# SvenGronauer/phoenix-drone-simulation

Measured on AMD Instinct MI355X. Metric: env-steps/sec, higher is better.
Workload: dtype f32; 1 GPU; DroneHoverSimpleEnv-v0, 1048576 envs per GPU lockstep, fp32, observation noise off, thrust noise 0, domain randomisation -1, auto-reset on, action ring [64,N,4] = hover+0.0 + 0.1*N(0,1); envs_per_gpu=1048576, obs_dim=42, bytes_per_env_step=346, parallelism=env-shard x1, no data-path collective

## Files before the change

### include/pds.h

```cpp
#ifndef PDS_H
#define PDS_H

#include <stdint.h>

#ifdef __cplusplus
extern "C" {
#endif

#define PDS_VERSION 2

#define PDS_TASK_HOVER 0
#define PDS_TASK_CIRCLE 1
#define PDS_TASK_TAKEOFF 2

#define PDS_CTRL_PWM 0
#define PDS_CTRL_ATTITUDE_RATE 1
#define PDS_CTRL_ATTITUDE 2

#define PDS_MAX_LATENCY_STEPS 8
#define PDS_MAX_REF_POINTS 300

#define PDS_OK 0
#define PDS_EINVAL -1
#define PDS_ENODEVICE -2
#define PDS_EHIP -3
#define PDS_ENOMEM -4
#define PDS_EUNSUPPORTED -5

typedef struct pds_config {
  int32_t struct_size;
  int32_t task;
  int64_t num_envs;
  int64_t env_id_base;
  uint64_t seed;
  int32_t device;
  int32_t use_motor_dynamics;
  int32_t use_ground_effect;
  int32_t observation_noise;
  int32_t aggregate_phy_steps;
  int32_t enable_reset_distribution;
  int32_t max_episode_steps;
  int32_t auto_reset;
// ... 107 lines not shown
int pds_latency_steps(const pds_handle *h);

int pds_field_width(int field);
int pds_get_state(pds_handle *h, int field, void *d_out, void *stream);
int pds_set_state(pds_handle *h, int field, const void *d_in, void *stream);

int pds_count_nonfinite(pds_handle *h, int64_t *count, void *stream);

uint64_t pds_tick(const pds_handle *h);
uint64_t pds_sync_tick(pds_handle *h, void *stream);
int pds_set_tick(pds_handle *h, uint64_t tick);

int pds_bytes_per_env_step(const pds_handle *h);
int pds_bytes_per_env_step_k(const pds_handle *h, int k_steps);

const char *pds_last_error(const pds_handle *h);

int pds_philox4x32(const uint32_t *d_ctr, const uint32_t *d_key, int rounds, int64_t n, uint32_t *d_out, void *stream);

int pds_noise_normals(uint64_t seed, uint64_t tick, uint32_t block, uint64_t env_id_base, int64_t n, float *d_out, void *stream);

int pds_history_advance(int64_t n, int half, int history, const float *d_obs2, const uint8_t *d_terminated,
                        const uint8_t *d_truncated, const float *d_final_obs2, int auto_reset, const float *d_hist_in,
                        float *d_hist_out, float *d_final_hist, void *stream);

int pds_gae(const float *d_rew, const float *d_val, const uint8_t *d_terminated, const uint8_t *d_truncated,
            const float *d_final_val, const float *d_last_val, float gamma, float lam, float rew_scale,
            float rew_clip, int64_t T, int64_t N, float *d_adv, float *d_target_v, float *d_disc_ret,
            void *stream);

// ... 75 lines not shown
```

### phoenix-drone-simulation_amd/csrc/pds_api.hip

```cpp
#include <hip/hip_runtime.h>

#include <cmath>
#include <cstdarg>
#include <cstdio>
#include <cstdlib>
#include <cstring>
#include <new>
#include <utility>
#include <vector>

#include "pds_reset.h"

namespace pds {

struct FieldArgs {
  DevState st;
  Consts k;
  void *user;
  long long n;
  int field;
  int task;
  int set;
  int has_motor, has_dr, has_tn, has_on, ctrl;
  int regen_obs;
// ... 202 lines not shown
  DevState st;
  Consts k;
  LaunchFlags flags;
  int force_tile;
  float2 *d_circle_ref;
  void *slab;
  float4 *lat_buf;
  unsigned long long *d_count;
  unsigned long long *d_stamps;
  int obs_dim;
  int num_cus;
  uint64_t tick;
  bool was_reset;
  int stored_from_agg;
  bool split_reset;
  bool stored_ready;
  char err[512];
};

struct DeviceGuard {
  int prev = -1;
  bool switched = false;
  hipError_t err = hipSuccess;
  explicit DeviceGuard(int dev) {
    err = hipGetDevice(&prev);
    if (err == hipSuccess && prev != dev) {
      err = hipSetDevice(dev);
      switched = err == hipSuccess;
    }
  }
// ... 225 lines not shown
  h->cfg = *cfg;
  fill_consts(*cfg, h->k);
  h->obs_dim = obs_dim_of(*cfg);
  h->flags.motor = cfg->use_motor_dynamics != 0;
  h->flags.dr = cfg->domain_randomization > 0;
  h->flags.ge = cfg->use_ground_effect != 0;
  h->flags.tn = cfg->motor_thrust_noise > 0;
  h->flags.on = cfg->observation_noise > 0;
  h->flags.ctrl = cfg->control_mode;
  h->flags.lat = lat_steps > 0;
  h->flags.hold = h->k.obs_rate != 1;
  h->flags.half_tile = false;
  if (const char *ft = getenv("PDS_FORCE_TILE")) h->force_tile = (ft[0] == 'h') ? 1 : ((ft[0] == 'f') ? 2 : 0);
  h->split_reset = false;
  if (const char *sr = getenv("PDS_SPLIT_RESET")) h->split_reset = sr[0] == '1';
  h->stored_from_agg = PDS_STORED_OH_FROM_AGG;
  if (PDS_STORED_OH_FROM_AGG > 0)
    if (const char *sa = getenv("PDS_STORED_OH_FROM_AGG")) h->stored_from_agg = atoi(sa);
  const size_t n = (size_t)cfg->num_envs;
  const size_t ntiles = (n + kWave - 1) / kWave;
  const LaunchFlags &f = h->flags;
  DeviceGuard guard(cfg->device);
  hipError_t e = guard.err;
  if (e == hipSuccess) {
    hipDeviceProp_t prop;
    e = hipGetDeviceProperties(&prop, cfg->device);
    h->num_cus = (e == hipSuccess && prop.multiProcessorCount > 0) ? prop.multiProcessorCount : 256;
  }
  std::vector<std::pair<void **, size_t>> req;
  auto alloc = [&](void **p, size_t bytes) { req.emplace_back(p, bytes); };
// ... 1 lines not shown
  alloc((void **)&h->st.hist[0], n * 16); alloc((void **)&h->st.hist[1], n * 16);
  alloc((void **)&h->st.ctr, n * 4);
  alloc((void **)&h->st.clk, ntiles * sizeof(WaveClock));
  alloc((void **)&h->d_count, 256);
  if (f.motor) alloc((void **)&h->st.mx, n * 16);
  if (f.dr) { alloc((void **)&h->st.par0, n * 16); alloc((void **)&h->st.par1, n * 8); }
  if (f.dr && f.motor) { alloc((void **)&h->st.mA, n * 16); alloc((void **)&h->st.mK, n * 16); }
  if (f.tn) alloc((void **)&h->st.ou, n * 16);
  if (f.on) {
    alloc((void **)&h->st.nz0, n * 16); alloc((void **)&h->st.nz1, n * 8);
    alloc((void **)&h->st.oh0, n * 16); alloc((void **)&h->st.oh1, n * 16); alloc((void **)&h->st.oh2, n * 8);
  }
  if (f.ctrl >= 1) { alloc((void **)&h->st.pid0, n * 16); alloc((void **)&h->st.pid1, n * 8); }
  if (f.ctrl == 2) { alloc((void **)&h->st.pid2, n * 16); alloc((void **)&h->st.pid3, n * 8); }
  alloc((void **)&h->d_circle_ref, kRefPoints * sizeof(float2));
  {
    const size_t stagger = (size_t)kStaggerBytes;
    size_t total = 0;
    std::vector<size_t> off;
    for (size_t j = 0; j < req.size(); ++j) {
      total = (total + 255) / 256 * 256 + stagger;
      off.push_back(total);
      total += req[j].second;
    }
    if (e == hipSuccess) e = hipMalloc(&h->slab, total + 256);
    if (e == hipSuccess) e = hipMemset(h->slab, 0, total + 256);
    if (e == hipSuccess)
      for (size_t j = 0; j < req.size(); ++j) *req[j].first = (char *)h->slab + off[j];
  }
  if (e == hipSuccess) {
    float2 ref[kRefPoints];
    const int np = h->k.ref_points;
    for (int t = 0; t < kRefPoints; ++t) {
      const double ts = 2 * M_PI * (double)(t % np) / np;
      ref[t].x = (float)(0.25 * (1 - cos(ts)));
      ref[t].y = (float)(0.25 * sin(ts));
    }
    e = hipMemcpy(h->d_circle_ref, ref, sizeof(ref), hipMemcpyHostToDevice);
  }
  h->st.circle_ref = h->d_circle_ref;
  if (e == hipSuccess && h->flags.on) {
    hipLaunchKernelGGL(ctor_noise_kernel, dim3((unsigned)((n + 255) / 256)), dim3(256), 0, 0, h->st, (long long)n,
                       (unsigned long long)cfg->env_id_base, h->k.gyro_sb, (uint32_t)cfg->seed, (uint32_t)(cfg->seed >> 32));
    e = hipGetLastError();
  }
  if (e == hipSuccess) e = hipDeviceSynchronize();
  if (e != hipSuccess) {
    snprintf(g_create_err, sizeof(g_create_err), "allocation of %zu envs failed: %s", n, hipGetErrorString(e));
    pds_destroy(h);
    return e == hipErrorOutOfMemory ? PDS_ENOMEM : PDS_EHIP;
  }
  if (h->flags.lat) {
    const int rc = ensure_latency_buffer(h);
    if (rc != PDS_OK) {
      snprintf(g_create_err, sizeof(g_create_err), "%s", h->err);
      pds_destroy(h);
      return rc;
    }
  }
  *out = h;
  return PDS_OK;
}

extern "C" int pds_destroy(pds_handle *h) {
  if (!h) return PDS_OK;
  DeviceGuard guard(h->cfg.device);
  if (h->slab) (void)hipFree(h->slab);
  if (h->lat_buf) (void)hipFree(h->lat_buf);
  if (h->d_stamps) (void)hipFree(h->d_stamps);
  delete h;
  return PDS_OK;
}

extern "C" int pds_obs_dim(const pds_handle *h) { return h ? h->obs_dim : PDS_EINVAL; }
extern "C" int64_t pds_num_envs(const pds_handle *h) { return h ? h->cfg.num_envs : PDS_EINVAL; }
extern "C" uint64_t pds_tick(const pds_handle *h) { return h ? h->tick : 0; }
extern "C" int pds_latency_steps(const pds_handle *h) { return h ? h->k.lat_steps : PDS_EINVAL; }
extern "C" const char *pds_last_error(const pds_handle *h) { return h ? h->err : g_create_err; }

extern "C" uint64_t pds_sync_tick(pds_handle *h, void *stream) {
  if (!h) return 0;
  DeviceGuard guard(h->cfg.device);
  WaveClock c;
  if (hipStreamSynchronize((hipStream_t)stream) == hipSuccess &&
      hipMemcpy(&c, h->st.clk, sizeof(c), hipMemcpyDeviceToHost) == hipSuccess)
    h->tick = ((uint64_t)c.y << 32) | c.x;
// ... 161 lines not shown
  const unsigned cus = (unsigned)h->num_cus;
  lf.half_tile = grid.x > (unsigned)kFullTileBlocksPerCU * cus * (256 / kBlock) && grid.x <= (merged ? 5u : 8u) * cus * (256 / kBlock);
  if (h->force_tile) lf.half_tile = h->force_tile == 1;
  if (lf.on || lf.lat) lf.half_tile = false;
  int kind = kLaunchStep;
  if (PDS_REGEN_OBS && h->stored_from_agg > 0 && lf.on && !lf.hold && h->cfg.aggregate_phy_steps >= h->stored_from_agg &&
      d_variates == nullptr) {
    kind = kLaunchStepStored;
    if (!h->stored_ready) {
      if (const int rc = materialize_kept_obs(h, (hipStream_t)stream)) return rc;
      h->stored_ready = true;
    }
  }
  const bool split = h->split_reset && h->cfg.auto_reset && d_variates == nullptr && kind == kLaunchStep &&
                     split_reset_supported(h->cfg.task, lf);
  launch_family(h, split ? kLaunchStepSplit : kind, lf, grid, (hipStream_t)stream, a);
  if (split) {
    a.k_steps = lf.hold ? 2 : ((PDS_REGEN_OBS && lf.on) ? 0 : 1);
    const dim3 pgrid((unsigned)((a.n + kPostResetEnvsPerBlock - 1) / kPostResetEnvsPerBlock));
    launch_family(h, kLaunchPostReset, lf, pgrid, (hipStream_t)stream, a);
  }
  PDS_HIP(h, hipGetLastError());
  h->tick += 1;
  return PDS_OK;
}

extern "C" int pds_step(pds_handle *h, const float *d_actions, float *d_obs, float *d_reward,
                        uint8_t *d_terminated, uint8_t *d_truncated, float *d_cost, float *d_final_obs,
                        void *stream) {
  return pds_step_with_variates(h, d_actions, nullptr, d_obs, d_reward, d_terminated, d_truncated, d_cost,
                                d_final_obs, stream);
// ... 178 lines not shown
  DeviceGuard guard(h->cfg.device);
  PDS_HIP(h, guard.err);
  FieldArgs a;
  memset(&a, 0, sizeof(a));
  a.st = h->st; a.k = h->k; a.user = d_ptr; a.n = h->cfg.num_envs; a.field = field; a.task = h->cfg.task; a.set = set;
  a.has_motor = h->flags.motor; a.has_dr = h->flags.dr; a.has_tn = h->flags.tn; a.has_on = h->flags.on; a.ctrl = h->flags.ctrl;
  a.regen_obs = PDS_REGEN_OBS && h->flags.on && !h->flags.hold;
  if (set && field != PDS_F_NOISY_OBS)
    if (const int rc = materialize_kept_obs(h, (hipStream_t)stream)) return rc;
  a.env_id_base = (unsigned long long)h->cfg.env_id_base;
  a.seed_lo = (uint32_t)h->cfg.seed; a.seed_hi = (uint32_t)(h->cfg.seed >> 32);
  const dim3 grid((unsigned)((a.n + kBlock - 1) / kBlock));
  hipLaunchKernelGGL(field_kernel, grid, dim3(kBlock), 0, (hipStream_t)stream, a);
  PDS_HIP(h, hipGetLastError());
  if (set) h->was_reset = true;
  return PDS_OK;
}

extern "C" int pds_count_nonfinite(pds_handle *h, int64_t *count, void *stream) {
  if (!h || !count) return PDS_EINVAL;
  DeviceGuard guard(h->cfg.device);
  PDS_HIP(h, guard.err);
  hipStream_t s = (hipStream_t)stream;
  PDS_HIP(h, hipMemsetAsync(h->d_count, 0, sizeof(*h->d_count), s));
  const long long n = h->cfg.num_envs;
  hipLaunchKernelGGL(nonfinite_kernel, dim3((unsigned)((n + 255) / 256)), dim3(256), 0, s, h->st, n, h->d_count);
  PDS_HIP(h, hipGetLastError());
  unsigned long long host = 0;
  PDS_HIP(h, hipMemcpyAsync(&host, h->d_count, sizeof(host), hipMemcpyDeviceToHost, s));
  PDS_HIP(h, hipStreamSynchronize(s));
  *count = (int64_t)host;
  return PDS_OK;
}

extern "C" int pds_get_state(pds_handle *h, int field, void *d_out, void *stream) { return do_field(h, field, d_out, 0, stream); }
extern "C" int pds_set_state(pds_handle *h, int field, const void *d_in, void *stream) { return do_field(h, field, const_cast<void *>(d_in), 1, stream); }

template <int ROUNDS>
__global__ __launch_bounds__(256) void philox_kernel(const uint32_t *ctr, const uint32_t *key, long long n, uint32_t *out) {
  const long long i = (long long)blockIdx.x * blockDim.x + threadIdx.x;
  if (i >= n) return;
  const U4 r = philox4x32<ROUNDS>(ctr[4 * i], ctr[4 * i + 1], ctr[4 * i + 2], ctr[4 * i + 3], key[2 * i], key[2 * i + 1]);
  out[4 * i] = r.x; out[4 * i + 1] = r.y; out[4 * i + 2] = r.z; out[4 * i + 3] = r.w;
}

__global__ __launch_bounds__(256) void noise_normals_kernel(uint32_t seed_lo, uint32_t seed_hi, uint32_t tick_lo, uint32_t tick_hi,
                                                            uint32_t block, unsigned long long id_base, long long n, float *out) {
// ... 53 lines not shown
```

### phoenix-drone-simulation_amd/csrc/pds_reset.h

```cpp
#pragma once
#include "pds_types.h"

namespace pds {

constexpr uint32_t kBlkReset = 0;
constexpr uint32_t kBlkLatRows = 9;
constexpr uint32_t kBlkResetNoise = 32;
constexpr uint32_t kBlkObsNoise = 64;
constexpr uint32_t kBlkSubNoise = 128;
constexpr uint32_t kBlkSubNoiseX = 256;

constexpr int kResetBlocks = 9;
constexpr int kObsCallBlocks = 3;
constexpr int kResetNoiseBlocks = 2 * kObsCallBlocks;
constexpr int kLatRowBlocks = kMaxLatSteps - 1;
constexpr int kScratchBlocks = kResetBlocks + kResetNoiseBlocks + kLatRowBlocks;

PDS_DEV void words_to_uniforms4(const U4 &w, float (&u)[4]) {
  u[0] = u01(w.x); u[1] = u01(w.y); u[2] = u01(w.z); u[3] = u01(w.w);
}
PDS_DEV void words_to_normals4(const U4 &w, float (&z)[4]) {
  box_muller(w.x, w.y, z[0], z[1]);
  box_muller(w.z, w.w, z[2], z[3]);
}
// ... 691 lines not shown
    float stale_w[3] = {0.f, 0.f, 0.f}, bias[3] = {0.f, 0.f, 0.f};
    if (V::ON) {
      const float4 q2 = a.st.s2[i];
      const float4 nz = a.st.nz0[i];
      stale_w[0] = q2.y; stale_w[1] = q2.z; stale_w[2] = q2.w;
      bias[0] = nz.x; bias[1] = nz.y; bias[2] = nz.z;
    }
    ResetOut r;
    const DirectWords dw((uint32_t)(a.env_id_base + (unsigned long long)i), rk);
    const uint32_t ctr_old = ctr_pack(0u, 0u, circle_ref_offset(a.st.ctr[i], a.k.ref_points));
    reset_compute<V>(a, ref_lds, dw, ctr_old, a.samples != nullptr ? a.samples + i * PDS_SAMPLE_FLOATS : nullptr,
                     stale_w, bias, r);
    reset_store<V>(a, ref_lds, i, r);
  }
  advance_clock(a.st.clk, tile, rk, parity, 1u, threadIdx.x & (kWave - 1));
}

template <class V>
__global__ __launch_bounds__(kWave) void post_reset_kernel(const StepArgs a) {
  constexpr int D = V::D;
  constexpr int kPer = kPostResetEnvsPerBlock / kWave;
  static_assert(kPer == 16 || kPer == 8 || kPer == 4, "one 16- / 8- / 4-byte load of each flag array per lane");
  __shared__ uint32_t queue[kPostResetEnvsPerBlock];
  __shared__ int qn;
  const float2 *ref_lds = nullptr;
  const int lane = threadIdx.x;
  const long long base = (long long)blockIdx.x * kPostResetEnvsPerBlock;
  if (lane == 0) qn = 0;
  __builtin_amdgcn_fence(__ATOMIC_RELEASE, "workgroup");
  __builtin_amdgcn_wave_barrier();
// ... 13 lines not shown
    } else {
      for (int j = 0; j < kPer; ++j)
        if (e0 + j < a.n && (a.term[e0 + j] | a.trunc[e0 + j])) fl[j >> 2] |= 1u << (8 * (j & 3));
    }
    if ((fl[0] | fl[1] | fl[2] | fl[3]) != 0u) {
      int cnt = 0;
      for (int j = 0; j < kPer; ++j) cnt += ((fl[j >> 2] >> (8 * (j & 3))) & 0xFFu) != 0u;
      int at_ = atomicAdd(&qn, cnt);
      for (int j = 0; j < kPer; ++j)
        if (((fl[j >> 2] >> (8 * (j & 3))) & 0xFFu) != 0u) queue[at_++] = (uint32_t)(kPer * lane + j);
    }
  }
  __builtin_amdgcn_fence(__ATOMIC_RELEASE, "workgroup");
  __builtin_amdgcn_wave_barrier();
  __builtin_amdgcn_fence(__ATOMIC_ACQUIRE, "workgroup");
  const int n_fin = __builtin_amdgcn_readfirstlane(qn);
  for (int idx = lane; idx < n_fin; idx += kWave) {
    const long long i = base + queue[idx];
    const WaveClock clk = a.st.clk[i / kWave];
    RngKey rk{a.seed_lo, a.seed_hi, 0u, 0u};
    {
      const unsigned long long t = (((unsigned long long)clk.y << 32) | clk.x) - 1ull;
      rk.tick_lo = (uint32_t)t; rk.tick_hi = (uint32_t)(t >> 32);
    }
    if (a.final_obs != nullptr) {
      const float2 *src = reinterpret_cast<const float2 *>(a.obs + i * D);
      float2 *dst = reinterpret_cast<float2 *>(a.final_obs + i * D);
#pragma unroll
      for (int j = 0; j < D / 2; ++j) dst[j] = src[j];
    }
    float stale_w[3] = {0.f, 0.f, 0.f}, bias[3] = {0.f, 0.f, 0.f};
    if (V::ON) {
      const float4 q2 = a.st.s2[i];
      const float4 nz = a.st.nz0[i];
      stale_w[0] = q2.y; stale_w[1] = q2.z; stale_w[2] = q2.w;
      bias[0] = nz.x; bias[1] = nz.y; bias[2] = nz.z;
    }
    uint32_t ref_offset = 0u;
    if (V::TASK == PDS_TASK_CIRCLE && !a.k.reset_dist) ref_offset = circle_ref_offset(a.st.ctr[i], a.k.ref_points);
    ResetOut r;
    const DirectWords dw((uint32_t)(a.env_id_base + (unsigned long long)i), rk);
    reset_compute<V>(a, ref_lds, dw, ctr_pack(0u, 0u, ref_offset), nullptr, stale_w, bias, r);
    reset_store<V>(a, ref_lds, i, r, a.k_steps);
  }
}

}
```

### phoenix-drone-simulation_amd/csrc/pds_step.h

```cpp
#pragma once
#include <type_traits>
#include "pds_reset.h"

namespace pds {

template <int D>
constexpr int tile_stride() {
  return (D % 8 == 0) ? D + 4 : D;
}

template <int HW>
constexpr int park_stride() {
  return (HW % 4 == 0) ? ((HW / 4) % 2 == 1 ? HW : HW + 4) : (HW % 2 == 1 ? HW : HW + 1);
}

template <int N>
PDS_DEV void lds_store_row(float *dst, const float *src) {
  static_assert(N % 4 == 0, "float4 rows");
#pragma unroll
  for (int j = 0; j < N / 4; ++j)
    reinterpret_cast<float4 *>(dst)[j] = make_float4(src[4 * j], src[4 * j + 1], src[4 * j + 2], src[4 * j + 3]);
}

template <class V>
// ... 594 lines not shown
      S.oh.qx = fresh ? S.oh.qx : held.qx; S.oh.qy = fresh ? S.oh.qy : held.qy; S.oh.qz = fresh ? S.oh.qz : held.qz;
      S.oh.qw = fresh ? S.oh.qw : held.qw;
      S.oh.vx = fresh ? S.oh.vx : held.vx; S.oh.vy = fresh ? S.oh.vy : held.vy; S.oh.vz = fresh ? S.oh.vz : held.vz;
    }
    put_noisy_half<TASK, O + 4, VEC>(row2, S.oh, ns.lpf, act, tx, ty, tz, pa2);
  } else {
    put_obs_half<TASK, O + 4, VEC>(row2, e, q, act, tx, ty, tz, pa2);
  }

  S.ctr = ctr_pack((uint32_t)(step + 1), 0u, (uint32_t)phase1, lat_idx);
  if (regen_obs_variant<V>() && a.noise != nullptr) S.ctr |= kCtrOhBit;
  S.h2 = h1;
  S.h1 = act;
  const bool need_reset = (V::SPLIT_RESET && STORE) ? false : (a.auto_reset && (done || trunc) && active);
  const unsigned long long reset_mask = __ballot(need_reset);
  const unsigned long long done_mask = (a.final_obs != nullptr || fin_lds != nullptr) ? reset_mask : 0ull;
  if (so != nullptr) { so->reward = reward; so->done = done; so->trunc = trunc; }
  bool was_reset = false;
  if (reset_mask != 0ull) {
    const int pos = __builtin_amdgcn_mbcnt_hi((uint32_t)(reset_mask >> 32), __builtin_amdgcn_mbcnt_lo((uint32_t)reset_mask, 0u));
    if constexpr (RM == RM_DEFERRED) {
      qcount = __popcll(reset_mask);
      if (need_reset) queue[pos] = (uint32_t)lane | ((uint32_t)ref_offset << 6);
    } else if constexpr (RM == RM_MERGED) {
      const StepArgs &a = reload_args<101, heavy_variant<V>()>(a_in, (int)o1);
      const int count = __popcll(reset_mask);
      if (need_reset) queue[pos] = (uint32_t)lane;
      __builtin_amdgcn_fence(__ATOMIC_RELEASE, "wavefront");
      __builtin_amdgcn_wave_barrier();
      __builtin_amdgcn_fence(__ATOMIC_ACQUIRE, "wavefront");
      float4 u0 = act, mxr = make_float4(xm[0], xm[1], xm[2], xm[3]);
// ... 189 lines not shown
  return was_reset;
}

#ifndef PDS_MIN_WAVES_LEAN
#define PDS_MIN_WAVES_LEAN 4
#endif
#ifndef PDS_MIN_WAVES
#define PDS_MIN_WAVES (V::ON ? (four_block_variant<V>() ? 4 : 3) : PDS_MIN_WAVES_LEAN)
#endif

template <class V, int TR>
constexpr bool inline_reset_single_step() {
  return TR == kWave && inline_single_step_rule(V::TASK, V::ON, V::LAT, V::CTRL);
}

#ifndef PDS_MERGED_HALF_PT1DR
#define PDS_MERGED_HALF_PT1DR 1
#endif
template <class V, int TR = kWave>
constexpr bool merged_reset_variant() {
  return PDS_MERGED_RESET && !V::ON && !V::LAT && V::TASK != PDS_TASK_TAKEOFF && (TR == kWave || !(V::MOTOR && V::DR) || (PDS_MERGED_HALF_PT1DR && V::CTRL == 0 && !V::TN));
}

#ifndef PDS_KERNARG_PREFETCH
#define PDS_KERNARG_PREFETCH 1
#endif
PDS_DEV void prefetch_kernargs() {
#if PDS_KERNARG_PREFETCH
  static_assert(sizeof(StepArgs) > 8 * 64 && sizeof(StepArgs) <= 9 * 64, "prefetch_kernargs touches lines 0..8: adjust");
  const auto p = __builtin_amdgcn_kernarg_segment_ptr();
// ... 47 lines not shown
#ifdef PDS_STAMPS
#define PDS_STAMP_ARG , stamp_
#define PDS_STAMP_DECL unsigned long long stamp_[kStampSlots] = {0, 0, 0, 0, 0, 0, 0, 0, 0, 0}; stamp_[0] = __builtin_amdgcn_s_memtime(); stamp_[8] = __builtin_amdgcn_s_memrealtime();
#define PDS_STAMP_FLUSH                                                                                \
  do {                                                                                                 \
    PDS_STAMP_WAIT(7);                                                                                 \
    stamp_[9] = __builtin_amdgcn_s_memrealtime();                                                      \
    if (a.stamps != nullptr && lane == 0)                                                              \
      for (int j_ = 0; j_ < kStampSlots; ++j_) a.stamps[t * kStampSlots + j_] = stamp_[j_];            \
  } while (0)
#else
#define PDS_STAMP_ARG
#define PDS_STAMP_DECL
#define PDS_STAMP_FLUSH do { } while (0)
#endif

template <class V, int TR>
__global__ __launch_bounds__(kBlock, (PDS_MIN_WAVES) * (256 / kBlock)) void step_kernel(const StepArgs a) {
  PDS_STAMP_DECL
  prefetch_kernargs();
  constexpr int RM = merged_reset_variant<V, TR>() ? RM_MERGED : (inline_reset_single_step<V, TR>() ? RM_INLINE : RM_DEFERRED);
  PDS_WAVE_SETUP(V, TR, RM, true)
  Loaded cur;
  load_env<V>(a, ix, t, cur);
  __builtin_amdgcn_sched_barrier(0);
  PDS_STAMP(1);
  PDS_STAMP_WAIT(2);
  RngKey rk{a.seed_lo, a.seed_hi, 0u, 0u};
  int parity;
  rk.tick_lo = (uint32_t)__builtin_amdgcn_readfirstlane((int)cur.clk.x);
  rk.tick_hi = (uint32_t)__builtin_amdgcn_readfirstlane((int)cur.clk.y);
  parity = __builtin_amdgcn_readfirstlane((int)cur.clk.z) & 1;
  EnvState S;
  unpack_state<V>(a.k, cur, parity, S);
  init_kept_obs<V>(a, rk, ix, S);
  int qcount = 0;
  step_once<V, TR, RM, true>(a, 0ll, rk, parity, ref_lds, tile, park, queue, scratch, lane, wave_base, ix, active, cur.act, S, qcount, nullptr, nullptr PDS_STAMP_ARG);
  if (RM == RM_DEFERRED && qcount > 0) {
    const float own_w[3] = {S.e.wx, S.e.wy, S.e.wz};
    drain_reset_queue<V>(reload_args<104, heavy_variant<V>()>(a), rk, ref_lds, queue, qcount, lane, wave_base, tile, own_w, S.ns.bias);
  }
  PDS_STAMP(6);
  advance_clock(reload_args<105, heavy_variant<V>()>(a).st.clk, t, rk, parity ^ 1, 1u, lane);
  PDS_STAMP_FLUSH;
}

#ifndef PDS_STEPK_OPAQUE_KEY
#define PDS_STEPK_OPAQUE_KEY 1
#endif
#ifndef PDS_STEPK_MIN_WAVES_OF
#define PDS_STEPK_MIN_WAVES_OF(V) 3
#endif
template <class V_>
__global__ __launch_bounds__(kBlock, (PDS_STEPK_MIN_WAVES_OF(V_)) * (256 / kBlock)) void step_k_kernel(const StepArgs a) {
  using W = std::conditional_t<regen_obs_variant<V_>(), StoredOh<V_>, V_>;
  constexpr int TR = kWave;
  constexpr int RM = merged_reset_variant<W>() ? RM_MERGED : RM_INLINE;
#ifdef PDS_STAMPS
// ... 47 lines not shown
  } else {
#if PDS_STORED_OH_FROM_AGG > 0
    if constexpr (regen_obs_variant<V>()) {
      if (kind == kLaunchStepStored) {
        hipLaunchKernelGGL((step_kernel<StoredOh<V>, kWave>), grid, dim3(kBlock), 0, s, a);
        return;
      }
    }
#endif
    if constexpr (!V::ON && !V::LAT) {
      if (half_tile) {
        hipLaunchKernelGGL((step_kernel<V, kHalfTileRows>), grid, dim3(kBlock), 0, s, a);
        return;
      }
    }
    if constexpr (inline_reset_single_step<V, kWave>()) {
      if (kind == kLaunchStepSplit) {
        hipLaunchKernelGGL((step_kernel<SplitReset<V>, kWave>), grid, dim3(kBlock), 0, s, a);
        return;
      }
    }
    hipLaunchKernelGGL((step_kernel<V, kWave>), grid, dim3(kBlock), 0, s, a);
  }
}

template <int TASK, int CTRL, bool LAT, bool HOLD, bool MOTOR, bool DR, bool GE, bool TN, bool ON>
struct MakeVariant {
  using type = Variant<TASK, MOTOR, DR, GE, TN, ON, CTRL, LAT, HOLD>;
};

// ... 80 lines not shown
```

### phoenix-drone-simulation_amd/csrc/pds_types.h

```cpp
#pragma once
#include <hip/hip_runtime.h>
#include <stddef.h>
#include <stdint.h>

#include "../../include/pds.h"
#include "pds_device.h"

namespace pds {

#ifndef PDS_BLOCK
#define PDS_BLOCK 256
#endif
constexpr int kBlock = PDS_BLOCK;
#ifndef PDS_MERGED_RESET
#define PDS_MERGED_RESET 1
#endif
constexpr int kWave = 64;
constexpr int kHalfTileRows = 32;
constexpr int kFullTileBlocksPerCU = 3;
constexpr int kQueueCap = 64;
constexpr int kRefPoints = 300;
constexpr int kStaggerBytes = 4352;

constexpr int kStampSlots = 10;
// ... 103 lines not shown
  int ref_points;
  float ref_dth_hi, ref_dth_lo;
  int obs_rate;
};

struct StepArgs {
  DevState st;
  Consts k;
  const float4 *actions;
  float *obs;
  float *reward;
  uint8_t *term;
  uint8_t *trunc;
  float *cost;
  float *final_obs;
  const uint8_t *mask;
  const float *samples;
  const float *noise;
  long long n;
  unsigned long long env_id_base;
  uint32_t seed_lo, seed_hi;
  int auto_reset;
  int k_steps;
  unsigned long long *stamps;
};

#ifndef PDS_RELOAD_ARGS
#define PDS_RELOAD_ARGS 1
#endif
template <int ID, bool ENABLE = true>
PDS_DEV const StepArgs &reload_args(const StepArgs &passed, int tag = 0) {
  if (!ENABLE || !PDS_RELOAD_ARGS) return passed;
// ... 10 lines not shown
struct Variant {
  static constexpr bool HOLD = HOLD_;
  static constexpr int CTRL = CTRL_;
  static constexpr bool LAT = LAT_;
  static constexpr int TASK = TASK_;
  static constexpr bool MOTOR = MOTOR_;
  static constexpr bool DR = DR_;
  static constexpr bool GE = GE_;
  static constexpr bool TN = TN_;
  static constexpr bool ON = ON_;
  static constexpr int O = ON_ ? (TASK_ == PDS_TASK_HOVER ? 13 : (TASK_ == PDS_TASK_CIRCLE ? 16 : 20))
                               : (TASK_ == PDS_TASK_HOVER ? 17 : (TASK_ == PDS_TASK_CIRCLE ? 16 : 20));
  static constexpr int D = 2 * (O + 4);
  static constexpr bool OH_STORED = false;
  static constexpr bool SPLIT_RESET = false;
};

template <class V>
struct StoredOh : V {
  static constexpr bool OH_STORED = true;
};

template <class V>
struct SplitReset : V {
  static constexpr bool SPLIT_RESET = true;
};

struct EnvRegs {
  float px, py, pz, vx, vy, vz, roll, pitch, yaw, wx, wy, wz;
};

struct Params {
  float dt, m, Jx, Jy, Jz, ftf1;
  float A[4], K[4];
};

struct ObsNoise {
  float pos_z[3], pos_u[3], vel_z[3], bias_z[3], rw_z[3], to_z[3], th_z[3], th_u[3];
};

// ... 53 lines not shown
  int ctrl;
  bool lat;
  bool hold;
  bool half_tile;
};
#ifndef PDS_STORED_OH_FROM_AGG
#define PDS_STORED_OH_FROM_AGG 0
#endif
#ifndef PDS_INLINE_SINGLE_STEP
#define PDS_INLINE_SINGLE_STEP 1
#endif
constexpr bool inline_single_step_rule(int task, bool on, bool lat, int ctrl) {
  return PDS_INLINE_SINGLE_STEP && (on || lat) && task != PDS_TASK_TAKEOFF && !(task == PDS_TASK_CIRCLE && (lat || ctrl != 0));
}
inline bool split_reset_supported(int task, const LaunchFlags &f) { return inline_single_step_rule(task, f.on, f.lat, f.ctrl); }
enum LaunchKind { kLaunchStep = 0, kLaunchStepK = 1, kLaunchReset = 2, kLaunchStepStored = 3, kLaunchStepSplit = 4, kLaunchPostReset = 5 };
#ifndef PDS_POST_RESET_ENVS
#define PDS_POST_RESET_ENVS 1024
#endif
constexpr int kPostResetEnvsPerBlock = PDS_POST_RESET_ENVS;
struct RolloutArgs {
  StepArgs s;
  pds_mlp pi, vf;
  const float *mean, *stdv;
  float eps;
  const float *log_std;
  unsigned long long seed;
  const unsigned long long *call_base;
  unsigned long long call_offset;
  int deterministic, T;
  const float *obs0;
  float *act_buf, *logp_buf, *val_buf, *fval_buf, *last_val;
  float *ep_ret, *ep_len, *stats;
};

// ... 62 lines not shown
```

### phoenix-drone-simulation_amd/envs.py

```python
import contextlib
import ctypes as C
import sys

import numpy as np
import torch

from . import native

_NULL_CTX = contextlib.nullcontext()

try:
    from gymnasium.spaces import Box as _GymBox
except Exception:
    _GymBox = None


_RAW_STREAM = getattr(torch._C, "_cuda_getCurrentRawStream", None)

class Box:

    def __init__(self, low, high, dtype=np.float32):
        self.low = np.asarray(low, dtype=dtype)
        self.high = np.asarray(high, dtype=dtype)
        self.shape = self.low.shape
# ... 369 lines not shown
    def set_state(self, name, value):
        fid = native.FIELDS[name]
        w = self.lib.pds_field_width(fid)
        dt = torch.int32 if name in native.INT_FIELDS else torch.float32
        v = torch.as_tensor(value).to(device=self.device, dtype=dt).reshape(self.num_envs, w).contiguous()
        rc = self.lib.pds_set_state(self._handle, fid, C.c_void_p(v.data_ptr()), self._stream())
        native.check(self._handle, rc, f"pds_set_state({name})")
        torch.cuda.current_stream(self.device).synchronize()

    def count_nonfinite(self):
        out = C.c_int64(0)
        rc = self.lib.pds_count_nonfinite(self._handle, C.byref(out), self._stream())
        native.check(self._handle, rc, "pds_count_nonfinite")
        return int(out.value)

    def state_dict(self):
        sd = {name: self.get_state(name) for name in native.FIELDS if name != "quat"}
        sd["tick"] = int(self.tick)
        if self._hist is not None:
            sd["observation_history"] = self._hist.clone()
        return sd

    def load_state_dict(self, sd):
        for name, v in sd.items():
            if name == "observation_history":
                self._hist = v.to(self.device).clone()
            elif name != "tick":
                self.set_state(name, v)
        rc = self.lib.pds_set_tick(self._handle, int(sd["tick"]))
        native.check(self._handle, rc, "pds_set_tick")
# ... 49 lines not shown
```

### phoenix-drone-simulation_amd/native.py

```python
import ctypes as C
import os

from .build import library_path

TASK_HOVER, TASK_CIRCLE, TASK_TAKEOFF = 0, 1, 2
OK, EINVAL, ENODEVICE, EHIP, ENOMEM, EUNSUPPORTED = 0, -1, -2, -3, -4, -5
SAMPLE_FLOATS = 112
MAX_LATENCY_STEPS = 8
NOISE_FLOATS = 52
FIELDS = dict(pos=0, rpy=1, vel=2, omega=3, quat=4, motor_x=5, last_action=6, prev_action=7,
              step_count=8, quat_sign=9, ref_offset=10, params=11, motor_A=12, motor_K=13, ou=14,
              gyro_bias=15, gyro_lpf=16, noisy_obs=17, pid=18, action_buffer=19, action_idx=20)
CONTROL_MODES = {'PWM': 0, 'AttitudeRate': 1, 'Attitude': 2}
INT_FIELDS = ("step_count", "quat_sign", "ref_offset", "action_idx")
SAMPLE_LAYOUT = dict(pos_offset=(0, 3), rpy=(3, 3), vel=(6, 3), omega=(9, 3), motor_x=(12, 4),
                     action=(16, 4), dr_dt=(20, 1), dr_m=(21, 1), dr_J=(22, 3), dr_ftf0=(25, 1),
                     dr_ftf1=(26, 1), dr_T=(27, 4), dr_t2w=(31, 4), ref_offset=(35, 1),
                     noise_call0=(36, 24), noise_call1=(60, 24), action_buf=(84, 28))
OBS_NOISE_LAYOUT = dict(pos_z=0, pos_u=3, vel_z=6, bias_z=9, rw_z=12, to_z=15, th_z=18, th_u=21)
STEP_NOISE_LAYOUT = dict(ou=0, a_bias=4, a_rw=7, a_to=10, obs=13, a_pos_z=37, a_pos_u=40, a_vel_z=43, a_th_z=46, a_th_u=49)

EXPORTS = ["pds_version", "pds_default_config", "pds_create", "pds_destroy", "pds_obs_dim",
           "pds_num_envs", "pds_reset", "pds_reset_from_samples", "pds_step", "pds_step_with_variates",
           "pds_field_width",
           "pds_get_state", "pds_set_state", "pds_tick", "pds_set_tick", "pds_sync_tick", "pds_count_nonfinite",
           "pds_bytes_per_env_step", "pds_bytes_per_env_step_k", "pds_last_error", "pds_step_k", "pds_set_latency",
           "pds_latency_steps", "pds_philox4x32", "pds_noise_normals", "pds_gae", "pds_history_advance",
           "pds_mlp_param_count", "pds_mlp_workspace_floats", "pds_mlp_forward", "pds_ppo_policy_grad",
           "pds_value_grad", "pds_ppo_policy_grad_step", "pds_value_grad_step", "pds_gaussian_sample", "pds_gaussian_sample_dev", "pds_counter_add", "pds_permutation", "pds_rollout_record",
           "pds_adam_step", "pds_rollout", "pds_rollout_history",
           "pds_npg_workspace_floats", "pds_npg_fisher_vector_product", "pds_npg_cg_step", "pds_npg_surrogate_kl"]


class Mlp(C.Structure):
    _fields_ = [("d_in", C.c_int32), ("h1", C.c_int32), ("h2", C.c_int32), ("d_out", C.c_int32),
                ("activation", C.c_int32),
                ("w1", C.c_void_p), ("b1", C.c_void_p), ("w2", C.c_void_p), ("b2", C.c_void_p),
                ("w3", C.c_void_p), ("b3", C.c_void_p)]


class Adam(C.Structure):
    _fields_ = [("d_exp_avg", C.c_void_p), ("d_exp_avg_sq", C.c_void_p), ("step", C.c_int64),
                ("lr", C.c_float), ("beta1", C.c_float), ("beta2", C.c_float), ("eps", C.c_float)]


class Config(C.Structure):
# ... 81 lines not shown

    later("pds_ppo_policy_grad_step", [mp, vp, vp, vp, vp, vp, i64, C.c_float, vp, vp, vp, ap, vp])
    later("pds_value_grad_step", [mp, vp, vp, vp, i64, vp, vp, vp, ap, vp])
    later("pds_gaussian_sample_dev", [vp, vp, i64, i32, u64, vp, u64, u64, i32, vp, vp, vp])
    later("pds_counter_add", [vp, u64, vp])
    later("pds_noise_normals", [u64, u64, C.c_uint32, u64, i64, vp, vp])
    later("pds_permutation", [vp, i64, u64, u64, vp])
    later("pds_rollout", [vp, i32, mp, mp, vp, vp, C.c_float, vp, u64, vp, u64, i32] + [vp] * 14)
    later("pds_rollout_history", [vp, i32, i32, mp, vp, vp, C.c_float, vp, u64, vp, u64, i32] + [vp] * 9 + [i32] + [vp] * 4)
    later("pds_npg_workspace_floats", [mp, i32])
    if hasattr(lib, "pds_npg_workspace_floats"):
        lib.pds_npg_workspace_floats.restype = i64
    later("pds_npg_fisher_vector_product", [mp, vp, vp, i64, vp, vp, C.c_float, vp, vp, vp])
    later("pds_npg_cg_step", [i64, vp, vp, vp, vp, vp, C.c_float, C.c_float, i32, vp])
    later("pds_npg_surrogate_kl", [mp, vp, vp, i32] + [vp] * 6 + [i64, vp, vp, vp, vp])
    _lib = lib
    return lib


def default_config(task):
    cfg = Config()
    rc = load().pds_default_config(int(task), C.byref(cfg))
    if rc != OK:
        raise ValueError(f"pds_default_config({task}) -> {rc}")
    return cfg


def check(handle, rc, what):
    if rc == OK:
        return
# ... 5 lines not shown
```

Before: 18.98 billion env-steps/s.

## Add group-wide deferred reset drained by last wave via cross-block counters

Adds a GroupReset step variant, on by default for hover tasks without latency or control. After stepping, each wave publishes its finished-env mask to global memory and bumps a per-group atomic counter, with dense waves resetting their own envs. One drainer wave per 1024-env group spins on the counter, collects the masks and resets all finished envs of the group. This moves the divergent reset work out of the hot step path and balances it across lanes, at the cost of inter-block polling, global atomics and a stall watchdog reported through pinned host memory.

```diff
diff --git a/include/pds.h b/include/pds.h
--- a/include/pds.h
+++ b/include/pds.h
@@ -26,6 +26,7 @@
 #define PDS_EHIP -3
 #define PDS_ENOMEM -4
 #define PDS_EUNSUPPORTED -5
+#define PDS_ESTALLED -6
 
 typedef struct pds_config {
   int32_t struct_size;
@@ -163,6 +164,8 @@
 int pds_bytes_per_env_step(const pds_handle *h);
 int pds_bytes_per_env_step_k(const pds_handle *h, int k_steps);
 
+uint32_t pds_device_status(const pds_handle *h);
+
 const char *pds_last_error(const pds_handle *h);
 
 int pds_philox4x32(const uint32_t *d_ctr, const uint32_t *d_key, int rounds, int64_t n, uint32_t *d_out, void *stream);
diff --git a/phoenix-drone-simulation_amd/csrc/pds_api.hip b/phoenix-drone-simulation_amd/csrc/pds_api.hip
--- a/phoenix-drone-simulation_amd/csrc/pds_api.hip
+++ b/phoenix-drone-simulation_amd/csrc/pds_api.hip
@@ -240,6 +240,9 @@
   bool was_reset;
   int stored_from_agg;
   bool split_reset;
+  bool group_reset;
+  uint32_t *group_sync;
+  volatile uint32_t *group_status;
   bool stored_ready;
   char err[512];
 };
@@ -495,6 +498,8 @@
   if (const char *ft = getenv("PDS_FORCE_TILE")) h->force_tile = (ft[0] == 'h') ? 1 : ((ft[0] == 'f') ? 2 : 0);
   h->split_reset = false;
   if (const char *sr = getenv("PDS_SPLIT_RESET")) h->split_reset = sr[0] == '1';
+  h->group_reset = PDS_GROUP_RESET_DEFAULT != 0;
+  if (const char *gr = getenv("PDS_GROUP_RESET")) h->group_reset = gr[0] == '1';
   h->stored_from_agg = PDS_STORED_OH_FROM_AGG;
   if (PDS_STORED_OH_FROM_AGG > 0)
     if (const char *sa = getenv("PDS_STORED_OH_FROM_AGG")) h->stored_from_agg = atoi(sa);
@@ -526,6 +531,7 @@
   if (f.ctrl >= 1) { alloc((void **)&h->st.pid0, n * 16); alloc((void **)&h->st.pid1, n * 8); }
   if (f.ctrl == 2) { alloc((void **)&h->st.pid2, n * 16); alloc((void **)&h->st.pid3, n * 8); }
   alloc((void **)&h->d_circle_ref, kRefPoints * sizeof(float2));
+  alloc((void **)&h->group_sync, group_sync_bytes((long long)n));
   {
     const size_t stagger = (size_t)kStaggerBytes;
     size_t total = 0;
@@ -551,6 +557,14 @@
     e = hipMemcpy(h->d_circle_ref, ref, sizeof(ref), hipMemcpyHostToDevice);
   }
   h->st.circle_ref = h->d_circle_ref;
+  if (e == hipSuccess) {
+    void *p = nullptr;
+    e = hipHostMalloc(&p, 64, hipHostMallocDefault);
+    if (e == hipSuccess) {
+      h->group_status = (volatile uint32_t *)p;
+      *h->group_status = 0u;
+    }
+  }
   if (e == hipSuccess && h->flags.on) {
     hipLaunchKernelGGL(ctor_noise_kernel, dim3((unsigned)((n + 255) / 256)), dim3(256), 0, 0, h->st, (long long)n,
                        (unsigned long long)cfg->env_id_base, h->k.gyro_sb, (uint32_t)cfg->seed, (uint32_t)(cfg->seed >> 32));
@@ -580,8 +594,20 @@
   if (h->slab) (void)hipFree(h->slab);
   if (h->lat_buf) (void)hipFree(h->lat_buf);
   if (h->d_stamps) (void)hipFree(h->d_stamps);
+  const bool stalled = h->group_status != nullptr && *h->group_status != 0u;
+  if (h->group_status) (void)hipHostFree((void *)h->group_status);
   delete h;
-  return PDS_OK;
+  return stalled ? PDS_ESTALLED : PDS_OK;
+}
+
+extern "C" uint32_t pds_device_status(const pds_handle *h) { return (h && h->group_status) ? *h->group_status : 0u; }
+
+static int group_status_check(pds_handle *h) {
+  const uint32_t w = pds_device_status(h);
+  if (w == 0u) return PDS_OK;
+  return fail(h, PDS_ESTALLED, "pds_step: the reset drainer of env group %u (envs %llu...) gave up waiting for the group's waves; "
+              "its finished envs were not reset (PDS_GROUP_RESET=0 selects the in-place reset)", w - 1u,
+              (unsigned long long)(w - 1u) * kPostResetEnvsPerBlock);
 }
 
 extern "C" int pds_obs_dim(const pds_handle *h) { return h ? h->obs_dim : PDS_EINVAL; }
@@ -773,7 +799,13 @@
   }
   const bool split = h->split_reset && h->cfg.auto_reset && d_variates == nullptr && kind == kLaunchStep &&
                      split_reset_supported(h->cfg.task, lf);
-  launch_family(h, split ? kLaunchStepSplit : kind, lf, grid, (hipStream_t)stream, a);
+  const bool group = !split && h->group_reset && h->cfg.auto_reset && d_variates == nullptr && kind == kLaunchStep &&
+                     group_reset_supported(h->cfg.task, lf);
+  if (group) {
+    a.group_sync = h->group_sync;
+    a.group_status = const_cast<uint32_t *>(h->group_status);
+  }
+  launch_family(h, split ? kLaunchStepSplit : (group ? kLaunchStepGroup : kind), lf, grid, (hipStream_t)stream, a);
   if (split) {
     a.k_steps = lf.hold ? 2 : ((PDS_REGEN_OBS && lf.on) ? 0 : 1);
     const dim3 pgrid((unsigned)((a.n + kPostResetEnvsPerBlock - 1) / kPostResetEnvsPerBlock));
@@ -982,7 +1014,7 @@
   hipLaunchKernelGGL(field_kernel, grid, dim3(kBlock), 0, (hipStream_t)stream, a);
   PDS_HIP(h, hipGetLastError());
   if (set) h->was_reset = true;
-  return PDS_OK;
+  return set ? PDS_OK : group_status_check(h);
 }
 
 extern "C" int pds_count_nonfinite(pds_handle *h, int64_t *count, void *stream) {
@@ -998,7 +1030,7 @@
   PDS_HIP(h, hipMemcpyAsync(&host, h->d_count, sizeof(host), hipMemcpyDeviceToHost, s));
   PDS_HIP(h, hipStreamSynchronize(s));
   *count = (int64_t)host;
-  return PDS_OK;
+  return group_status_check(h);
 }
 
 extern "C" int pds_get_state(pds_handle *h, int field, void *d_out, void *stream) { return do_field(h, field, d_out, 0, stream); }
diff --git a/phoenix-drone-simulation_amd/csrc/pds_reset.h b/phoenix-drone-simulation_amd/csrc/pds_reset.h
--- a/phoenix-drone-simulation_amd/csrc/pds_reset.h
+++ b/phoenix-drone-simulation_amd/csrc/pds_reset.h
@@ -729,6 +729,40 @@
     reset_store<V>(a, ref_lds, i, r);
   }
   advance_clock(a.st.clk, tile, rk, parity, 1u, threadIdx.x & (kWave - 1));
+}
+
+template <class V, bool COPY_FINAL>
+PDS_DEV void post_reset_serve(const StepArgs &a, const float2 *ref_lds, long long base, const uint32_t *queue, int n_fin, int lane,
+                              int oh_mode) {
+  constexpr int D = V::D;
+  for (int idx = lane; idx < n_fin; idx += kWave) {
+    const long long i = base + queue[idx];
+    const WaveClock clk = a.st.clk[i / kWave];
+    RngKey rk{a.seed_lo, a.seed_hi, 0u, 0u};
+    {
+      const unsigned long long t = (((unsigned long long)clk.y << 32) | clk.x) - 1ull;
+      rk.tick_lo = (uint32_t)t; rk.tick_hi = (uint32_t)(t >> 32);
+    }
+    if (COPY_FINAL && a.final_obs != nullptr) {
+      const float2 *src = reinterpret_cast<const float2 *>(a.obs + i * D);
+      float2 *dst = reinterpret_cast<float2 *>(a.final_obs + i * D);
+#pragma unroll
+      for (int j = 0; j < D / 2; ++j) dst[j] = src[j];
+    }
+    float stale_w[3] = {0.f, 0.f, 0.f}, bias[3] = {0.f, 0.f, 0.f};
+    if (V::ON) {
+      const float4 q2 = a.st.s2[i];
+      const float4 nz = a.st.nz0[i];
+      stale_w[0] = q2.y; stale_w[1] = q2.z; stale_w[2] = q2.w;
+      bias[0] = nz.x; bias[1] = nz.y; bias[2] = nz.z;
+    }
+    uint32_t ref_offset = 0u;
+    if (V::TASK == PDS_TASK_CIRCLE && !a.k.reset_dist) ref_offset = circle_ref_offset(a.st.ctr[i], a.k.ref_points);
+    ResetOut r;
+    const DirectWords dw((uint32_t)(a.env_id_base + (unsigned long long)i), rk);
+    reset_compute<V>(a, ref_lds, dw, ctr_pack(0u, 0u, ref_offset), nullptr, stale_w, bias, r);
+    reset_store<V>(a, ref_lds, i, r, oh_mode);
+  }
 }
 
 template <class V>
@@ -772,35 +806,7 @@
   __builtin_amdgcn_fence(__ATOMIC_RELEASE, "workgroup");
   __builtin_amdgcn_wave_barrier();
   __builtin_amdgcn_fence(__ATOMIC_ACQUIRE, "workgroup");
-  const int n_fin = __builtin_amdgcn_readfirstlane(qn);
-  for (int idx = lane; idx < n_fin; idx += kWave) {
-    const long long i = base + queue[idx];
-    const WaveClock clk = a.st.clk[i / kWave];
-    RngKey rk{a.seed_lo, a.seed_hi, 0u, 0u};
-    {
-      const unsigned long long t = (((unsigned long long)clk.y << 32) | clk.x) - 1ull;
-      rk.tick_lo = (uint32_t)t; rk.tick_hi = (uint32_t)(t >> 32);
-    }
-    if (a.final_obs != nullptr) {
-      const float2 *src = reinterpret_cast<const float2 *>(a.obs + i * D);
-      float2 *dst = reinterpret_cast<float2 *>(a.final_obs + i * D);
-#pragma unroll
-      for (int j = 0; j < D / 2; ++j) dst[j] = src[j];
-    }
-    float stale_w[3] = {0.f, 0.f, 0.f}, bias[3] = {0.f, 0.f, 0.f};
-    if (V::ON) {
-      const float4 q2 = a.st.s2[i];
-      const float4 nz = a.st.nz0[i];
-      stale_w[0] = q2.y; stale_w[1] = q2.z; stale_w[2] = q2.w;
-      bias[0] = nz.x; bias[1] = nz.y; bias[2] = nz.z;
-    }
-    uint32_t ref_offset = 0u;
-    if (V::TASK == PDS_TASK_CIRCLE && !a.k.reset_dist) ref_offset = circle_ref_offset(a.st.ctr[i], a.k.ref_points);
-    ResetOut r;
-    const DirectWords dw((uint32_t)(a.env_id_base + (unsigned long long)i), rk);
-    reset_compute<V>(a, ref_lds, dw, ctr_pack(0u, 0u, ref_offset), nullptr, stale_w, bias, r);
-    reset_store<V>(a, ref_lds, i, r, a.k_steps);
-  }
-}
-
-}
+  post_reset_serve<V, true>(a, ref_lds, base, queue, __builtin_amdgcn_readfirstlane(qn), lane, a.k_steps);
+}
+
+}
diff --git a/phoenix-drone-simulation_amd/csrc/pds_step.h b/phoenix-drone-simulation_amd/csrc/pds_step.h
--- a/phoenix-drone-simulation_amd/csrc/pds_step.h
+++ b/phoenix-drone-simulation_amd/csrc/pds_step.h
@@ -632,7 +632,9 @@
   S.h1 = act;
   const bool need_reset = (V::SPLIT_RESET && STORE) ? false : (a.auto_reset && (done || trunc) && active);
   const unsigned long long reset_mask = __ballot(need_reset);
-  const unsigned long long done_mask = (a.final_obs != nullptr || fin_lds != nullptr) ? reset_mask : 0ull;
+  constexpr bool kGroupForm = V::GROUP_RESET && STORE;
+  const unsigned long long fin_rows = kGroupForm ? __ballot(a.auto_reset && (done || trunc) && active) : reset_mask;
+  const unsigned long long done_mask = (a.final_obs != nullptr || fin_lds != nullptr) ? fin_rows : 0ull;
   if (so != nullptr) { so->reward = reward; so->done = done; so->trunc = trunc; }
   bool was_reset = false;
   if (reset_mask != 0ull) {
@@ -852,6 +854,11 @@
   return TR == kWave && inline_single_step_rule(V::TASK, V::ON, V::LAT, V::CTRL);
 }
 
+template <class V>
+constexpr bool group_reset_variant() {
+  return group_reset_rule(V::TASK, V::ON, V::LAT, V::CTRL, V::HOLD);
+}
+
 #ifndef PDS_MERGED_HALF_PT1DR
 #define PDS_MERGED_HALF_PT1DR 1
 #endif
@@ -929,6 +936,94 @@
 #define PDS_STAMP_DECL
 #define PDS_STAMP_FLUSH do { } while (0)
 #endif
+
+template <class V, int LDS_WORDS>
+PDS_DEV void group_reset_tail(const StepArgs &a, long long tile_index, long long ntiles, int lane, bool fin, uint32_t *lds) {
+  static_assert(LDS_WORDS > kPostResetEnvsPerBlock, "the queue of a group + its count live in the wave's observation tile");
+  constexpr int GT = kGroupTiles, WPB = kBlock / kWave, BPG = GT / WPB;
+  using RV = Variant<V::TASK, V::MOTOR, V::DR, false, false, V::ON, 0, V::LAT, false>;
+  const int oh_mode = V::HOLD ? 2 : ((PDS_REGEN_OBS && V::ON) ? 0 : 1);
+  const unsigned long long fin_mask = __ballot(fin);
+  const int n_own = __popcll(fin_mask);
+  const uint32_t t = (uint32_t)__builtin_amdgcn_readfirstlane((int)tile_index);
+  const uint32_t nt = (uint32_t)ntiles;
+  const uint32_t g = t / GT, blk = t / WPB, blk0 = g * BPG;
+  const uint32_t nb = gridDim.x, b = blockIdx.x;
+  const int nblk = (int)min((uint32_t)BPG, nb - blk0), j_own = (int)(blk - blk0);
+  bool last_block = j_own == nblk - 1;
+  if (PDS_XCD_REMAP && nb % 8u == 0u) {
+    const int per = (int)(nb / 8u);
+    last_block = true;
+    for (int j = 0; j < nblk; ++j) {
+      int y = (int)(b / 8u) + (j - j_own), x = (int)(b % 8u);
+      while (y >= per) { y -= per; ++x; }
+      while (y < 0) { y += per; --x; }
+      if ((uint32_t)(8 * y + x) > b) last_block = false;
+    }
+  }
+  const int tiles_here = (int)min((uint32_t)GT, nt - g * GT);
+  const bool drainer = last_block && (t % WPB) == min((uint32_t)(WPB - 1), nt - 1u - blk * WPB);
+  uint32_t *const counter = a.group_sync + (size_t)g * kGroupCounterStride;
+  unsigned long long *const masks =
+      reinterpret_cast<unsigned long long *>(a.group_sync + (size_t)((nt + GT - 1) / GT) * kGroupCounterStride) + (size_t)g * GT;
+  unsigned long long m = 0ull;
+  long long base;
+  if (!drainer) {
+    const bool dense = n_own >= kGroupDenseFrom;
+    if (n_own != 0 && !dense) {
+      if (lane == 0) masks[t % GT] = fin_mask;
+      asm volatile("s_waitcnt vmcnt(0)" ::: "memory");
+      __builtin_amdgcn_fence(__ATOMIC_RELEASE, "agent");
+      asm volatile("s_waitcnt vmcnt(0)" ::: "memory");
+    }
+    if (lane == 0) (void)__hip_atomic_fetch_add(counter, 1u, __ATOMIC_RELAXED, __HIP_MEMORY_SCOPE_AGENT);
+    if (!dense) return;
+    asm volatile("s_waitcnt vmcnt(0)" ::: "memory");
+    if (lane == 0) m = fin_mask;
+    base = (long long)t * kWave;
+  } else {
+    const uint32_t expected = (uint32_t)tiles_here - 1u;
+    uint32_t seen = 0u;
+    for (int it = 0; expected != 0u; ++it) {
+      seen = (uint32_t)__builtin_amdgcn_readfirstlane((int)__hip_atomic_load(counter, __ATOMIC_RELAXED, __HIP_MEMORY_SCOPE_AGENT));
+      if (seen >= expected) break;
+      if (it >= kGroupPollCap) {
+        if (lane == 0) __hip_atomic_store(a.group_status, g + 1u, __ATOMIC_RELAXED, __HIP_MEMORY_SCOPE_SYSTEM);
+        return;
+      }
+      __builtin_amdgcn_s_sleep(8);
+    }
+    __builtin_amdgcn_fence(__ATOMIC_ACQUIRE, "agent");
+    asm volatile("s_waitcnt vmcnt(0)" ::: "memory");
+    if (lane < tiles_here) {
+      if (lane == (int)(t % GT)) {
+        m = fin_mask;
+      } else {
+        m = __hip_atomic_load(masks + lane, __ATOMIC_RELAXED, __HIP_MEMORY_SCOPE_AGENT);
+        if (m != 0ull) masks[lane] = 0ull;
+      }
+    }
+    if (lane == 0 && expected != 0u) *counter = 0u;
+    base = (long long)g * kPostResetEnvsPerBlock;
+  }
+  uint32_t *const qn = lds + kPostResetEnvsPerBlock;
+  if (lane == 0) *qn = 0u;
+  __builtin_amdgcn_fence(__ATOMIC_RELEASE, "wavefront");
+  __builtin_amdgcn_wave_barrier();
+  __builtin_amdgcn_fence(__ATOMIC_ACQUIRE, "wavefront");
+  if (m != 0ull) {
+    uint32_t at_ = atomicAdd(qn, (uint32_t)__popcll(m));
+    while (m != 0ull) {
+      lds[at_++] = (uint32_t)(lane * kWave + __builtin_ctzll(m));
+      m &= m - 1ull;
+    }
+  }
+  __builtin_amdgcn_fence(__ATOMIC_RELEASE, "wavefront");
+  __builtin_amdgcn_wave_barrier();
+  __builtin_amdgcn_fence(__ATOMIC_ACQUIRE, "wavefront");
+  const int n_fin = __builtin_amdgcn_readfirstlane((int)*qn);
+  post_reset_serve<RV, false>(a, nullptr, base, lds, n_fin, lane, oh_mode);
+}
 
 template <class V, int TR>
 __global__ __launch_bounds__(kBlock, (PDS_MIN_WAVES) * (256 / kBlock)) void step_kernel(const StepArgs a) {
@@ -950,13 +1045,20 @@
   unpack_state<V>(a.k, cur, parity, S);
   init_kept_obs<V>(a, rk, ix, S);
   int qcount = 0;
-  step_once<V, TR, RM, true>(a, 0ll, rk, parity, ref_lds, tile, park, queue, scratch, lane, wave_base, ix, active, cur.act, S, qcount, nullptr, nullptr PDS_STAMP_ARG);
+  StepOut out_;
+  step_once<V, TR, RM, true>(a, 0ll, rk, parity, ref_lds, tile, park, queue, scratch, lane, wave_base, ix, active, cur.act, S, qcount, nullptr, V::GROUP_RESET ? &out_ : nullptr PDS_STAMP_ARG);
   if (RM == RM_DEFERRED && qcount > 0) {
     const float own_w[3] = {S.e.wx, S.e.wy, S.e.wz};
     drain_reset_queue<V>(reload_args<104, heavy_variant<V>()>(a), rk, ref_lds, queue, qcount, lane, wave_base, tile, own_w, S.ns.bias);
   }
   PDS_STAMP(6);
   advance_clock(reload_args<105, heavy_variant<V>()>(a).st.clk, t, rk, parity ^ 1, 1u, lane);
+  if constexpr (V::GROUP_RESET) {
+    static_assert(TR == kWave && RM == RM_INLINE, "the GroupReset form exists for the variants that reset in place on the full tile");
+    const StepArgs &g = reload_args<106, heavy_variant<V>()>(a);
+    group_reset_tail<V, TR * tile_stride<V::D>()>(g, t, ntiles, lane, g.auto_reset && (out_.done || out_.trunc) && active,
+                                                  reinterpret_cast<uint32_t *>(tile));
+  }
   PDS_STAMP_FLUSH;
 }
 
@@ -1034,6 +1136,12 @@
         return;
       }
     }
+    if constexpr (group_reset_variant<V>()) {
+      if (kind == kLaunchStepGroup) {
+        hipLaunchKernelGGL((step_kernel<GroupReset<V>, kWave>), grid, dim3(kBlock), 0, s, a);
+        return;
+      }
+    }
     if constexpr (inline_reset_single_step<V, kWave>()) {
       if (kind == kLaunchStepSplit) {
         hipLaunchKernelGGL((step_kernel<SplitReset<V>, kWave>), grid, dim3(kBlock), 0, s, a);
diff --git a/phoenix-drone-simulation_amd/csrc/pds_types.h b/phoenix-drone-simulation_amd/csrc/pds_types.h
--- a/phoenix-drone-simulation_amd/csrc/pds_types.h
+++ b/phoenix-drone-simulation_amd/csrc/pds_types.h
@@ -141,8 +141,14 @@
   uint8_t *trunc;
   float *cost;
   float *final_obs;
-  const uint8_t *mask;
-  const float *samples;
+  union {
+    const uint8_t *mask;
+    uint32_t *group_sync;
+  };
+  union {
+    const float *samples;
+    uint32_t *group_status;
+  };
   const float *noise;
   long long n;
   unsigned long long env_id_base;
@@ -183,6 +189,7 @@
   static constexpr int D = 2 * (O + 4);
   static constexpr bool OH_STORED = false;
   static constexpr bool SPLIT_RESET = false;
+  static constexpr bool GROUP_RESET = false;
 };
 
 template <class V>
@@ -193,6 +200,11 @@
 template <class V>
 struct SplitReset : V {
   static constexpr bool SPLIT_RESET = true;
+};
+
+template <class V>
+struct GroupReset : SplitReset<V> {
+  static constexpr bool GROUP_RESET = true;
 };
 
 struct EnvRegs {
@@ -276,11 +288,30 @@
   return PDS_INLINE_SINGLE_STEP && (on || lat) && task != PDS_TASK_TAKEOFF && !(task == PDS_TASK_CIRCLE && (lat || ctrl != 0));
 }
 inline bool split_reset_supported(int task, const LaunchFlags &f) { return inline_single_step_rule(task, f.on, f.lat, f.ctrl); }
-enum LaunchKind { kLaunchStep = 0, kLaunchStepK = 1, kLaunchReset = 2, kLaunchStepStored = 3, kLaunchStepSplit = 4, kLaunchPostReset = 5 };
+enum LaunchKind { kLaunchStep = 0, kLaunchStepK = 1, kLaunchReset = 2, kLaunchStepStored = 3, kLaunchStepSplit = 4, kLaunchPostReset = 5,
+                  kLaunchStepGroup = 6 };
 #ifndef PDS_POST_RESET_ENVS
 #define PDS_POST_RESET_ENVS 1024
 #endif
 constexpr int kPostResetEnvsPerBlock = PDS_POST_RESET_ENVS;
+
+constexpr bool group_reset_rule(int task, bool on, bool lat, int ctrl, bool hold) {
+  return inline_single_step_rule(task, on, lat, ctrl) && task == PDS_TASK_HOVER && !lat && ctrl == 0 && !hold;
+}
+inline bool group_reset_supported(int task, const LaunchFlags &f) { return group_reset_rule(task, f.on, f.lat, f.ctrl, f.hold); }
+#ifndef PDS_GROUP_RESET_DEFAULT
+#define PDS_GROUP_RESET_DEFAULT 1
+#endif
+constexpr int kGroupTiles = kPostResetEnvsPerBlock / kWave;
+static_assert(kGroupTiles >= kBlock / kWave && kGroupTiles <= kWave && kGroupTiles % (kBlock / kWave) == 0, "whole blocks; one mask per lane");
+#ifndef PDS_GROUP_DENSE_FROM
+#define PDS_GROUP_DENSE_FROM 16
+#endif
+constexpr int kGroupDenseFrom = PDS_GROUP_DENSE_FROM;
+constexpr int kGroupPollCap = 1 << 20;
+constexpr int kGroupCounterStride = 16;
+__host__ __device__ inline long long group_count(long long n) { return (n + kPostResetEnvsPerBlock - 1) / kPostResetEnvsPerBlock; }
+__host__ __device__ inline size_t group_sync_bytes(long long n) { return (size_t)group_count(n) * kGroupCounterStride * 4 + (size_t)((n + kWave - 1) / kWave) * 8; }
 struct RolloutArgs {
   StepArgs s;
   pds_mlp pi, vf;
diff --git a/phoenix-drone-simulation_amd/envs.py b/phoenix-drone-simulation_amd/envs.py
--- a/phoenix-drone-simulation_amd/envs.py
+++ b/phoenix-drone-simulation_amd/envs.py
@@ -407,6 +407,9 @@
         native.check(self._handle, rc, "pds_count_nonfinite")
         return int(out.value)
 
+    def device_status(self):
+        return int(self.lib.pds_device_status(self._handle))
+
     def state_dict(self):
         sd = {name: self.get_state(name) for name in native.FIELDS if name != "quat"}
         sd["tick"] = int(self.tick)
diff --git a/phoenix-drone-simulation_amd/native.py b/phoenix-drone-simulation_amd/native.py
--- a/phoenix-drone-simulation_amd/native.py
+++ b/phoenix-drone-simulation_amd/native.py
@@ -29,7 +29,8 @@
            "pds_mlp_param_count", "pds_mlp_workspace_floats", "pds_mlp_forward", "pds_ppo_policy_grad",
            "pds_value_grad", "pds_ppo_policy_grad_step", "pds_value_grad_step", "pds_gaussian_sample", "pds_gaussian_sample_dev", "pds_counter_add", "pds_permutation", "pds_rollout_record",
            "pds_adam_step", "pds_rollout", "pds_rollout_history",
-           "pds_npg_workspace_floats", "pds_npg_fisher_vector_product", "pds_npg_cg_step", "pds_npg_surrogate_kl"]
+           "pds_npg_workspace_floats", "pds_npg_fisher_vector_product", "pds_npg_cg_step", "pds_npg_surrogate_kl",
+           "pds_device_status"]
 
 
 class Mlp(C.Structure):
@@ -141,6 +142,9 @@
     later("pds_npg_fisher_vector_product", [mp, vp, vp, i64, vp, vp, C.c_float, vp, vp, vp])
     later("pds_npg_cg_step", [i64, vp, vp, vp, vp, vp, C.c_float, C.c_float, i32, vp])
     later("pds_npg_surrogate_kl", [mp, vp, vp, i32] + [vp] * 6 + [i64, vp, vp, vp, vp])
+    later("pds_device_status", [vp])
+    if hasattr(lib, "pds_device_status"):
+        lib.pds_device_status.restype = C.c_uint32
     _lib = lib
     return lib
 
```

Measured after the change: 18.98 billion env-steps/s (median of 4 runs). About the same (-0.0%).
